# loop-Z/omniisaacgymenvs_loop

Hardware: AMD Instinct MI355X
Metric: env-steps/sec USV_CaptureXY at 1/2/4/8 MI355X; wall-clock to reward=30 (higher is better)
Workload: dtype fp32; 1 GPU; USV_Virtual_CaptureXY num_envs=131072/GPU PPO-MLP fp32 (BASELINE configs[4] per GPU: 2^20 envs over 8 GPUs); num_envs_per_gpu=131072, horizon_length=16, minibatch_size=8192, mini_epochs=8, parallelism=dp1, exchange=none (one rank), seed=0, full=False

## Files before the change

omniisaacgymenvs_loop_amd/csrc/ppo.hip:

```cpp
#include <cstdlib>
#include <cstring>
#include <type_traits>

#include "usv_device.h"

USV_PROBE_DEFINE(ppo)
USV_PROBE_DEFINE(pol)
USV_PROBE_DEFINE(red)

namespace {

constexpr int NIN = PPO_NIN, NH = PPO_NH, NA = PPO_NA;
constexpr int RB = 32;
constexpr int TB = 256;
constexpr int XS = 35;
constexpr int HS = 129;
constexpr int NPART = PPO_NPARAM + 8;
constexpr int NPART_PAD = (NPART + 3) & ~3;
constexpr int P_LOSS = PPO_NPARAM;
constexpr float kLog2Pi = 1.8378770664093453f;

typedef float f32x16 __attribute__((ext_vector_type(16)));
typedef unsigned int u32x4_t __attribute__((ext_vector_type(4)));

// ... 831 lines not shown
    double *o = part + ((size_t)mb * OM_CH + ch) * 2 * NIN;
    o[tid] = t;
    o[NIN + tid] = t2;
  }
}

constexpr int RS_TB = 256, RS_U = 8;
__global__ __launch_bounds__(RS_TB) void k_obs_rms_seq(ppo_cfg_t c, const double *__restrict__ part, int nmb,
                                                       double *obs_rms, double *seq) {
  const double rows = (double)c.minibatch;
  for (int q = threadIdx.x; q < nmb * NIN; q += RS_TB) {
    const int mb = q / NIN, k = q % NIN;
    double sa = 0, sb = 0;
#pragma unroll
    for (int ch = 0; ch < OM_CH; ++ch) {
      const double *o = part + ((size_t)mb * OM_CH + ch) * 2 * NIN;
      sa += o[k];
      sb += o[NIN + k];
    }
    const double bmean = sa / rows;
    seq[(size_t)mb * 2 * NIN + k] = bmean;
    seq[(size_t)mb * 2 * NIN + NIN + k] = (sb - rows * bmean * bmean) / (rows - 1.0);
  }
  __syncthreads();
  const int k = threadIdx.x;
  if (k < NIN) {
    double mean = obs_rms[k], var = obs_rms[NIN + k], count = obs_rms[2 * NIN];
    for (int mb0 = 0; mb0 < nmb; mb0 += RS_U) {
      double bm[RS_U], bv[RS_U];
#pragma unroll
      for (int u = 0; u < RS_U; ++u) {
        const int mb = min(mb0 + u, nmb - 1);
        bm[u] = seq[(size_t)mb * 2 * NIN + k];
        bv[u] = seq[(size_t)mb * 2 * NIN + NIN + k];
      }
#pragma unroll
      for (int u = 0; u < RS_U; ++u) {
        if (mb0 + u >= nmb) break;
        const double tot = count + rows;
        const double delta = bm[u] - mean;
        const double M2 = var * count + bv[u] * rows + delta * delta * count * rows / tot;
        mean = mean + delta * rows / tot;
        var = M2 / tot;
        count = tot;
        seq[(size_t)(mb0 + u) * 2 * NIN + k] = mean;
        seq[(size_t)(mb0 + u) * 2 * NIN + NIN + k] = var;
      }
    }
    obs_rms[k] = mean;
    obs_rms[NIN + k] = var;
    if (k == 0) obs_rms[2 * NIN] = count;
  }
}

constexpr int GTB = 512;
#ifndef USV_BWD_SYNC
#define USV_BWD_SYNC 0
#endif
#ifndef USV_BWD_PRIO
#define USV_BWD_PRIO 0
#endif

#ifndef USV_RD_P
#define USV_RD_P 128
#endif
#ifndef USV_RD_NT
#define USV_RD_NT 1
#endif
typedef float f32x4v __attribute__((ext_vector_type(4)));
constexpr int RD_TB = 512, RD_P = USV_RD_P;
constexpr int RD_L = RD_P / 4;
constexpr int RD_G = (RD_TB / RD_L);
constexpr int RD_KB = 16;
constexpr int RED_BLOCKS = (PPO_NPARAM + 5 + RD_P - 1) / RD_P;
static_assert(RD_P % 4 == 0 && 64 % RD_L == 0 && RD_P <= RD_TB, "reduce geometry");
static_assert(RED_BLOCKS <= 256, "chunk squares: one per thread of waves 0-3");

struct AdamBanks {
  const float *P0, *m0, *v0;
  float *P1, *m1, *v1;
};
struct AdamK {
  float step_size, bc2s;
};
__device__ __forceinline__ AdamK adam_consts(const ppo_cfg_t &c, float lr, float step) {
  const double bc1 = 1.0 - pow((double)c.adam_b1, (double)step);
  const double bc2 = 1.0 - pow((double)c.adam_b2, (double)step);
  return {(float)((double)lr / bc1), (float)sqrt(bc2)};
}
__device__ __forceinline__ void adam_one(const ppo_cfg_t &c, const AdamK &k, float g, float p_old, float m_old,
                                         float v_old, float &pn, float &mn, float &vn) {
  if (c.weight_decay != 0.f) g = g + c.weight_decay * p_old;
  mn = m_old + (1.0f - c.adam_b1) * (g - m_old);
  vn = v_old * c.adam_b2 + (1.0f - c.adam_b2) * g * g;
  const float denom = sqrtf(vn) / k.bc2s + c.adam_eps;
  pn = p_old - k.step_size * (mn / denom);
}
__device__ __forceinline__ float clip_coef(const ppo_cfg_t &c, float total_norm) {
  float coef = 1.0f;
  if (c.truncate_grads) {
    coef = c.grad_norm / (total_norm + 1e-6f);
    coef = fminf(coef, 1.0f);
  }
  return coef;
}
__device__ __forceinline__ AdamK adam_consts_tagged(const ppo_cfg_t &c, float lr, float step, float t_ss,
                                                    float t_bc, float t_step, float t_lr) {
  if (t_step == step && t_lr == lr) return {t_ss, t_bc};
  return adam_consts(c, lr, step);
}
struct OptNext {
  float nl, kl_keep, step;
  AdamK nk;
};
template <class OptIn>
__device__ __forceinline__ OptNext opt_next(const ppo_cfg_t &c, const OptIn &opt_in, float kl) {
  const float lr = opt_in[0];
  float nl = lr, kl_keep = opt_in[2];
  if (c.lr_adaptive) {
    if (kl > 2.0f * c.kl_threshold) nl = fmaxf(lr / 1.5f, c.lr_min);
    if (kl < 0.5f * c.kl_threshold) nl = fminf(lr * 1.5f, c.lr_max);
    kl_keep = kl;
  }
  const float step = opt_in[1] + 1.0f;
  return {nl, kl_keep, step, adam_consts(c, nl, step + 1.0f)};
}
__device__ __forceinline__ void opt_store(const ppo_cfg_t &c, const OptNext &x, float *opt_out, float total_norm,
                                          float kl, float *kl_out) {
  if (c.lr_adaptive && kl_out) *kl_out = kl;
  opt_out[0] = x.nl;
  opt_out[1] = x.step;
  opt_out[2] = x.kl_keep;
  opt_out[3] = total_norm;
  opt_out[4] = x.nk.step_size;
  opt_out[5] = x.nk.bc2s;
  opt_out[6] = x.step + 1.0f;
  opt_out[7] = x.nl;
}

struct ChainIn {
  const float *P_prev, *m_prev, *v_prev;
  float *P_cur, *m_cur, *v_cur;
  const float *grad;
  const float *opt_prev;
  float *opt_cur;
  float *kl_out;
  uint32_t *dp_clock;
  int fold_skip;
  float gscale;
};

constexpr int XG = XS;
constexpr int GX = ((RB * XG + GTB - 1) / GTB) * GTB;
struct GradSmem {
  float w2[NH * HS];
  float w1[NH * XG];
  float x[GX];
  float h1[RB * HS];
  float h2[RB * HS];
  float xch[4][16][64];
  float out[RB * 4];
  float g[RB * 4];
  float hg[4][4][NH];
  float b1[NH];
  float tail[TAIL + 1];
  float nrm[4];
  int fold[2];
};

constexpr int S_W2 = 0, S_W1 = NH * NH, S_SIG = S_W1 + NH * 32, S_B1 = S_SIG + 2, S_TAIL = S_B1 + NH,
              S_W1C = S_TAIL + TAIL, S_END = S_W1C + NH;
static_assert(S_END == PPO_NPARAM && S_W1 % 4 == 0 && NIN == 33, "partial slot layout");
__device__ __forceinline__ int tail_slot(int param) { return S_TAIL + param - PPO_OFF_B2; }
__device__ __forceinline__ int acc_slot(int base, int tile, int a, int lane) { return base + ((tile * 4 + a) * 64 + lane) * 4; }
__device__ __forceinline__ int param_of_slot(int s) {
  if (s < S_W1) {
    const int tile = s >> 10, a = (s >> 8) & 3, lane = (s >> 2) & 63, q = 4 * a + (s & 3);
    const int n = 32 * (tile >> 2) + crow(q, lane >> 5), k = 32 * (tile & 3) + (lane & 31);
    return PPO_OFF_W2 + n * NH + k;
  }
  if (s < S_SIG) {
    const int t = s - S_W1, tile = t >> 10, a = (t >> 8) & 3, lane = (t >> 2) & 63, q = 4 * a + (t & 3);
    const int n = 32 * tile + crow(q, lane >> 5), k = lane & 31;
    return PPO_OFF_W1 + n * NIN + k;
  }
  if (s < S_B1) return PPO_OFF_SIGMA + (s - S_SIG);
  if (s < S_TAIL) return PPO_OFF_B1 + (s - S_B1);
  if (s < S_W1C) return PPO_OFF_B2 + (s - S_TAIL);
  if (s < S_END) return PPO_OFF_W1 + (s - S_W1C) * NIN + (NIN - 1);
  return -1;
}

#ifndef USV_ROW_NT
#define USV_ROW_NT 0
#endif
__device__ __forceinline__ float row_ld(const float *p) {
  if constexpr (USV_ROW_NT != 0) return __builtin_nontemporal_load(p);
  else return *p;
}
struct RowIn {
  float act0, act1, nlp, val, ret, adv, mu0, mu1, sg0, sg1;
};

#ifndef USV_PART_AUX
#define USV_PART_AUX 2
#endif
template <int kAux, bool kCM>
struct PartOutT {
  __amdgpu_buffer_rsrc_t r;
  uint32_t cs;
  __device__ __forceinline__ uint32_t off(int idx) const {
    if constexpr (kCM) return (uint32_t)(idx / RD_P) * cs + (uint32_t)(idx % RD_P) * 4u;
    else return (uint32_t)idx * 4u;
  }
  __device__ __forceinline__ void operator()(int idx, float v) const {
    __builtin_amdgcn_raw_buffer_store_b32(__builtin_bit_cast(uint32_t, v), r, off(idx), 0, kAux);
  }
  __device__ __forceinline__ void x4(int idx, float a, float b, float c, float d) const {
    const u32x4_t v = {__builtin_bit_cast(uint32_t, a), __builtin_bit_cast(uint32_t, b), __builtin_bit_cast(uint32_t, c),
                       __builtin_bit_cast(uint32_t, d)};
    __builtin_amdgcn_raw_buffer_store_b128(v, r, off(idx), 0, kAux);
  }
};
#ifndef USV_PART_CM
#define USV_PART_CM 1
#endif
constexpr int AUX_SC1 = 16;

constexpr int FOLD_G = 8;
static_assert(RD_G >= FOLD_G, "k_reduce_partials(fold = 1) reads one group row per row group");
constexpr int FOLD_MAX_M = 32;
constexpr int FOLD_CTL_STRIDE = 64;
constexpr uint64_t FOLD_WAIT_TICKS = 10000;
__host__ __device__ constexpr size_t part_body_floats(int nblk) {
  return (size_t)nblk * RED_BLOCKS * RD_P > (size_t)(nblk + FOLD_G) * NPART_PAD ? (size_t)nblk * RED_BLOCKS * RD_P
                                                                                 : (size_t)(nblk + FOLD_G) * NPART_PAD;
}
__device__ __forceinline__ uint32_t *fold_ctl(float *partials, int nblk) {
  return reinterpret_cast<uint32_t *>(partials + part_body_floats(nblk));
}
__device__ __forceinline__ const uint32_t *fold_ctl(const float *partials, int nblk) {
  return reinterpret_cast<const uint32_t *>(partials + part_body_floats(nblk));
}
__device__ __forceinline__ f32x4v ld4_sc1(__amdgpu_buffer_rsrc_t r, uint32_t byte_off) {
  return __builtin_bit_cast(f32x4v, __builtin_amdgcn_raw_buffer_load_b128(r, byte_off, 0, AUX_SC1));
}

__device__ __forceinline__ void redo_step(const ppo_cfg_t &c, const ChainIn &ch, const float (&op)[8], float coef,
                                          float scale, GradSmem &s, float &ls0, float &ls1) {
  const AdamK ak = adam_consts_tagged(c, op[0], op[1] + 1.0f, op[4], op[5], op[6], op[7]);
  for (int q = threadIdx.x; q < PPO_NPARAM; q += GTB) {
    float pn, mn, vn;
    adam_one(c, ak, ch.grad[q] * scale * coef, ch.P_prev[q], ch.m_prev[q], ch.v_prev[q], pn, mn, vn);
    if ((q / GTB) % gridDim.x == blockIdx.x) {
      ch.P_cur[q] = pn; ch.m_cur[q] = mn; ch.v_cur[q] = vn;
    }
    if (q >= PPO_OFF_B2) {
      s.tail[q - PPO_OFF_B2] = pn;
    } else if (q >= PPO_OFF_W2) {
      const int e = q - PPO_OFF_W2;
      s.w2[(e / NH) * HS + e % NH] = pn;
    } else if (q >= PPO_OFF_B1) {
      s.b1[q - PPO_OFF_B1] = pn;
    } else if (q >= PPO_OFF_W1) {
      const int e = q - PPO_OFF_W1;
      s.w1[(e / NIN) * XG + e % NIN] = pn;
    }
  }
  float pn, mn, vn;
  adam_one(c, ak, ch.grad[PPO_OFF_SIGMA] * scale * coef, ch.P_prev[PPO_OFF_SIGMA], ch.m_prev[PPO_OFF_SIGMA],
           ch.v_prev[PPO_OFF_SIGMA], pn, mn, vn);
  ls0 = pn;
  adam_one(c, ak, ch.grad[PPO_OFF_SIGMA + 1] * scale * coef, ch.P_prev[PPO_OFF_SIGMA + 1],
           ch.m_prev[PPO_OFF_SIGMA + 1], ch.v_prev[PPO_OFF_SIGMA + 1], pn, mn, vn);
  ls1 = pn;
}

constexpr int APN_TB = 256;
__device__ __forceinline__ float apply_norm_part(const float *__restrict__ grad_in, float grad_scale, int tid) {
  constexpr int N4 = PPO_NPARAM / 4, U = (N4 + APN_TB - 1) / APN_TB;
  const float4 *g4 = reinterpret_cast<const float4 *>(grad_in);
  float4 gv[U];
#pragma unroll
  for (int u = 0; u < U; ++u) gv[u] = g4[min(tid + u * APN_TB, N4 - 1)];
  float ss = 0.f;
#pragma unroll
  for (int u = 0; u < U; ++u) {
    if (tid + u * APN_TB >= N4) continue;
    const float x = gv[u].x * grad_scale, y = gv[u].y * grad_scale;
    const float z = gv[u].z * grad_scale, w = gv[u].w * grad_scale;
    ss = fmaf(x, x, ss); ss = fmaf(y, y, ss); ss = fmaf(z, z, ss); ss = fmaf(w, w, ss);
  }
  for (int r = 4 * N4 + tid; r < PPO_NPARAM; r += APN_TB) {
    const float g = grad_in[r] * grad_scale;
    ss = fmaf(g, g, ss);
  }
  return ss;
}

template <bool kBf, bool kChain, bool kFold, bool kColl = false>
__device__ __forceinline__ void mb_grad8w(const ppo_cfg_t &c, const ChainIn &ch, const float *__restrict__ P,
                                          const double *__restrict__ obs_rms, int row0,
                                          const float *__restrict__ e_obs, const float *__restrict__ e_act,
                                          const float *__restrict__ e_nlp, const float *__restrict__ e_val,
                                          const float *__restrict__ e_ret, const float *__restrict__ e_adv,
                                          float *e_mu, float *e_sigma, float *partials, GradSmem &s) {
  const int tid = threadIdx.x, lane = tid & 63, w = tid >> 6;
  const int i = lane & 31, h = lane >> 5;
  const int kh = w >> 2, cb = w & 3, n0 = 32 * cb;
#ifdef USV_DIAG_HOT_ROWS
  const int rb0 = blockIdx.x * RB;
#else
  const int rb0 = row0 + blockIdx.x * RB;
#endif
  const float invB = 1.0f / (float)c.minibatch;
  USV_PHASE(ppo, 0);
  if (ch.dp_clock && blockIdx.x == 0 && tid == 0) *ch.dp_clock += 1u;
  constexpr int NW1G = (NH * XG + GTB - 1) / GTB, NTLG = (TAIL + GTB - 1) / GTB, NW2F = NH * NH / GTB;
  static_assert(NH * NH % GTB == 0, "staging trip counts");
  float w2f[NW2F];
  float w1r[NW1G], tlr[NTLG];
  float ov = 0.f;
  if constexpr (kChain) ov = lane < 8 ? ch.opt_prev[lane] : ch.grad[PPO_NPARAM];
  {
#pragma unroll
    for (int u = 0; u < NW1G; ++u) {
      const int q = min(tid + u * GTB, NH * XG - 1), j = q / XG, k = q % XG;
      w1r[u] = P[PPO_OFF_W1 + j * NIN + min(k, NIN - 1)];
    }
#pragma unroll
    for (int u = 0; u < NTLG; ++u) tlr[u] = P[PPO_OFF_B2 + min(tid + u * GTB, TAIL - 1)];
  }
  const float b1r = P[PPO_OFF_B1 + (tid & (NH - 1))];
  const float lsv = P[PPO_OFF_SIGMA + (lane & 1)];
  float lsig0 = 0.f, lsig1 = 0.f;
  float csq = 0.f;
  if constexpr (kChain) csq = ch.grad[PPO_NPARAM + 8 + min(tid, RED_BLOCKS - 1)];
  RowIn ri;
  {
    const size_t row = (size_t)rb0 + (lane & (RB - 1));
    ri.act0 = row_ld(&e_act[row * 2]); ri.act1 = row_ld(&e_act[row * 2 + 1]);
    ri.nlp = row_ld(&e_nlp[row]); ri.adv = row_ld(&e_adv[row]);
    ri.val = row_ld(&e_val[row]); ri.ret = row_ld(&e_ret[row]);
    ri.mu0 = row_ld(&e_mu[row * 2]); ri.mu1 = row_ld(&e_mu[row * 2 + 1]);
    ri.sg0 = row_ld(&e_sigma[row * 2]); ri.sg1 = row_ld(&e_sigma[row * 2 + 1]);
  }
  constexpr int NU = (RB * XG + GTB - 1) / GTB;
  float xo[NU];
  double mu[NU], var[NU];
#pragma unroll
  for (int u = 0; u < NU; ++u) {
    const int q = min(tid + u * GTB, RB * XG - 1), r = q / XG, kc = min(q % XG, NIN - 1);
    xo[u] = row_ld(&e_obs[(size_t)(rb0 + r) * NIN + kc]);
    mu[u] = obs_rms[kc];
    var[u] = obs_rms[NIN + kc];
  }
#pragma unroll
  for (int u = 0; u < NW2F; ++u) w2f[u] = P[PPO_OFF_W2 + tid + u * GTB];
  __builtin_amdgcn_sched_barrier(0);
#pragma unroll
  for (int u = 0; u < NW1G; ++u)
    if ((tid + u * GTB) % XG >= NIN) w1r[u] = 0.f;
  if (kChain && tid >= RED_BLOCKS) csq = 0.f;
  {
    const bool norm = c.normalize_input != 0;
#pragma unroll
    for (int u = 0; u < NU; ++u) {
      const int q = tid + u * GTB;
      const int k = q % XG;
      const float xn = rms_norm(xo[u], mu[u], var[u], c.rms_eps);
      const float xv = (k < NIN && q < RB * XG) ? (norm ? xn : xo[u]) : 0.f;
      s.x[q] = xv;
    }
  }
#pragma unroll
  for (int u = 0; u < NW1G; ++u)
    if (tid + u * GTB < NH * XG) s.w1[tid + u * GTB] = w1r[u];
#pragma unroll
  for (int u = 0; u < NTLG; ++u)
    if (tid + u * GTB < TAIL) s.tail[tid + u * GTB] = tlr[u];
  if (tid < NH) s.b1[tid] = b1r;
  if (kChain && !kColl && w < 4) {
    const float t = wave_sum(csq);
    if (lane == 0) s.nrm[w] = t;
  }
  __syncthreads();
  if constexpr (kColl) {
    if (w < 4) {
      const float t = wave_sum(apply_norm_part(ch.grad, ch.gscale, tid));
      if (lane == 0) s.nrm[w] = t;
    }
    __syncthreads();
  }
  bool slow = false;
  if constexpr (kChain) {
    const auto lane_of = [&](int q) {
      return __builtin_bit_cast(float, __builtin_amdgcn_readlane(__builtin_bit_cast(int, ov), q));
    };
    const float total_norm = sqrtf(((s.nrm[0] + s.nrm[1]) + s.nrm[2]) + s.nrm[3]);
    const float coef = clip_coef(c, total_norm);
    const float gscale = kColl ? ch.gscale : 1.0f;
    if (blockIdx.x == 0 && tid == 256) {
      float op[8];
#pragma unroll
      for (int q = 0; q < 8; ++q) op[q] = lane_of(q);
      const float kl_prev = kColl ? lane_of(8) * gscale : lane_of(8);
      opt_store(c, opt_next(c, op, kl_prev), ch.opt_cur, total_norm, kl_prev, ch.kl_out);
    }
    if (kColl || coef < 1.0f) {
      slow = true;
      float op[8];
#pragma unroll
      for (int q = 0; q < 8; ++q) op[q] = lane_of(q);
      redo_step(c, ch, op, coef, gscale, s, lsig0, lsig1);
      __syncthreads();
    }
  }
  USV_PHASE(ppo, 1);
  if (kh == 0) {
    f32x16 acc = {};
#pragma unroll
    for (int st = 0; st < 17; ++st) {
      const int k = 2 * st + h;
      acc = mfma32(s.x[i * XG + k], s.w1[(n0 + i) * XG + k], acc);
    }
    const float bj = s.b1[n0 + i];
#pragma unroll
    for (int r = 0; r < 16; ++r) s.h1[crow(r, h) * HS + n0 + i] = fast_tanh(acc[r] + bj);
  }
  USV_PHASE(ppo, 9);
  if (!slow) {
#pragma unroll
    for (int u = 0; u < NW2F; ++u) {
      const int e = tid + u * GTB;
      s.w2[(e >> 7) * HS + (e & (NH - 1))] = w2f[u];
    }
  }
  __syncthreads();
  USV_PHASE(ppo, 10);
  const int ra = (i + 16 * kh) & (RB - 1);
  {
    f32x16 acc = {};
    if constexpr (kBf) {
#pragma unroll
      for (int st = 0; st < NH / 32; ++st) {
        const int k0 = 64 * kh + 16 * st + 8 * h;
        acc = mfma_bf16(ld8(&s.h1[ra * HS + k0]), ld8(&s.w2[(n0 + i) * HS + k0]), acc);
      }
    } else {
#pragma unroll 16
      for (int st = 0; st < NH / 4; ++st) {
        const int k = 64 * kh + 2 * st + h;
        acc = mfma32(s.h1[ra * HS + k], s.w2[(n0 + i) * HS + k], acc);
      }
    }
    USV_PHASE(ppo, 11);
#pragma unroll
    for (int q = 0; q < 8; ++q) s.xch[cb][8 * kh + q][lane] = acc[8 + q];
    __syncthreads();
    const float bj = s.tail[T_B2 + n0 + i];
#pragma unroll
    for (int q = 0; q < 8; ++q)
      s.h2[(crow(q, h) + 16 * kh) * HS + n0 + i] = fast_tanh((acc[q] + s.xch[cb][8 - 8 * kh + q][lane]) + bj);
  }
  __syncthreads();
  USV_PHASE(ppo, 12);
  constexpr bool kCM = USV_PART_CM != 0 && !kFold;
  const PartOutT<kFold ? AUX_SC1 : USV_PART_AUX, kCM> part_st{
      kCM ? __builtin_amdgcn_make_buffer_rsrc(partials + (size_t)blockIdx.x * RD_P, 0,
                                              (int)(((size_t)RED_BLOCKS * gridDim.x - blockIdx.x) * RD_P * 4), 0x00020000)
          : __builtin_amdgcn_make_buffer_rsrc(partials + (size_t)blockIdx.x * NPART_PAD, 0, NPART * 4, 0x00020000),
      (uint32_t)gridDim.x * RD_P * 4u};
  {
    const int r = tid / 16, part = tid % 16;
    float a0 = 0.f, a1 = 0.f, av = 0.f;
#pragma unroll
    for (int kk = 0; kk < 8; ++kk) {
      const int k = part + 16 * kk;
      const float hv = s.h2[r * HS + k];
      a0 = fmaf(s.tail[T_WMU + k], hv, a0);
      a1 = fmaf(s.tail[T_WMU + NH + k], hv, a1);
      av = fmaf(s.tail[T_WV + k], hv, av);
    }
#pragma unroll
    for (int m = 1; m < 16; m <<= 1) {
      a0 += __shfl_xor(a0, m, 64);
      a1 += __shfl_xor(a1, m, 64);
      av += __shfl_xor(av, m, 64);
    }
    if (part == 0) {
      s.out[r * 4 + 0] = a0 + s.tail[T_BMU];
      s.out[r * 4 + 1] = a1 + s.tail[T_BMU + 1];
      s.out[r * 4 + 2] = av + s.tail[T_BV];
    }
  }
  __syncthreads();
  USV_PHASE(ppo, 2);
  if (tid < 192) {
    const int r = lane;
    const bool rowok = r < RB;
    const int rr = rowok ? r : 0;
    const size_t row = (size_t)rb0 + rr;
    const float mu0 = s.out[rr * 4], mu1 = s.out[rr * 4 + 1], v = s.out[rr * 4 + 2];
    if (!slow) {
      lsig0 = __builtin_bit_cast(float, __builtin_amdgcn_readlane(__builtin_bit_cast(int, lsv), 0));
      lsig1 = __builtin_bit_cast(float, __builtin_amdgcn_readlane(__builtin_bit_cast(int, lsv), 1));
    }
    const float ls0 = mu0 * 0.f + lsig0, ls1 = mu1 * 0.f + lsig1;
    const float sg0 = expf(ls0), sg1 = expf(ls1);
    const float bh0 = fmaxf(mu0 - 1.1f, 0.f), bl0 = fminf(mu0 + 1.1f, 0.f);
    const float bh1 = fmaxf(mu1 - 1.1f, 0.f), bl1 = fminf(mu1 + 1.1f, 0.f);
    if (w == 0) {
      float la = 0.f, gs0 = 0.f, gs1 = 0.f;
      if (rowok) {
        const float z0 = (ri.act0 - mu0) / sg0, z1 = (ri.act1 - mu1) / sg1;
        const float nlp = 0.5f * (z0 * z0 + z1 * z1) + kLog2Pi + (ls0 + ls1);
        const float A = ri.adv;
        const float ratio = expf(ri.nlp - nlp);
        const float lo = 1.0f - c.e_clip, hi = 1.0f + c.e_clip;
        const float rc = clampt(ratio, lo, hi);
        const float s1 = -(A * ratio), s2 = -(A * rc);
        const float a_loss = fmaxf(s1, s2);
        const float inr = (ratio >= lo && ratio <= hi) ? 1.f : 0.f;
        const float g1 = -A, g2 = -A * inr;
        const float g_r = (s1 > s2) ? g1 : ((s1 < s2) ? g2 : 0.5f * (g1 + g2));
        const float dnlp = invB * g_r * (-ratio);
        const float bc = c.bounds_loss_coef * invB;
        const float dmu0 = dnlp * (-z0 / sg0) + bc * 2.f * (bh0 + bl0);
        const float dmu1 = dnlp * (-z1 / sg1) + bc * 2.f * (bh1 + bl1);
        const float dent = -c.entropy_coef * invB;
        gs0 = dnlp * (1.f - z0 * z0) + dent;
        gs1 = dnlp * (1.f - z1 * z1) + dent;
        la = a_loss;
        s.g[r * 4 + 0] = dmu0;
        s.g[r * 4 + 1] = dmu1;
        s.g[r * 4 + 3] = dnlp;
      }
      la = wave_sum(la); gs0 = wave_sum(gs0); gs1 = wave_sum(gs1);
      if (lane == 0) {
        part_st(P_LOSS + 0, la);
        part_st(S_SIG, gs0); part_st(S_SIG + 1, gs1);
      }
    } else if (w == 2) {
      float le = 0.f, lb = 0.f, lkl = 0.f;
      if (rowok) {
        const float b_loss = (bl0 * bl0 + bh0 * bh0) + (bl1 * bl1 + bh1 * bh1);
        const float ent = (0.5f + 0.5f * logf(USV_2PI_F) + ls0) + (0.5f + 0.5f * logf(USV_2PI_F) + ls1);
        const float om0 = ri.mu0, om1 = ri.mu1, os0 = ri.sg0, os1 = ri.sg1;
        const float kl0 = logf(os0 / sg0 + 1e-5f) + (sg0 * sg0 + (om0 - mu0) * (om0 - mu0)) / (2.0f * (os0 * os0 + 1e-5f)) - 0.5f;
        const float kl1 = logf(os1 / sg1 + 1e-5f) + (sg1 * sg1 + (om1 - mu1) * (om1 - mu1)) / (2.0f * (os1 * os1 + 1e-5f)) - 0.5f;
        e_mu[row * 2] = mu0; e_mu[row * 2 + 1] = mu1;
        e_sigma[row * 2] = sg0; e_sigma[row * 2 + 1] = sg1;
        le = ent; lb = b_loss; lkl = kl0 + kl1;
      }
      le = wave_sum(le); lb = wave_sum(lb); lkl = wave_sum(lkl);
      if (lane == 0) {
        part_st(P_LOSS + 2, le); part_st(P_LOSS + 3, lb); part_st(P_LOSS + 4, lkl);
      }
    } else {
      float lc = 0.f;
      if (rowok) {
        const float vo = ri.val, R = ri.ret;
        float dv, c_loss;
        if (c.clip_value) {
          const float dvr = v - vo;
          const float dvc = clampt(dvr, -c.e_clip, c.e_clip);
          const float vc = vo + dvc;
          const float l1 = (v - R) * (v - R), l2 = (vc - R) * (vc - R);
          c_loss = fmaxf(l1, l2);
          const float d1 = 2.f * (v - R);
          const float d2 = 2.f * (vc - R) * ((dvr >= -c.e_clip && dvr <= c.e_clip) ? 1.f : 0.f);
          dv = (l1 > l2) ? d1 : ((l1 < l2) ? d2 : 0.5f * (d1 + d2));
        } else {
          c_loss = (R - v) * (R - v);
          dv = 2.f * (v - R);
        }
        dv *= 0.5f * c.critic_coef * invB;
        lc = c_loss;
        s.g[r * 4 + 2] = dv;
      }
      lc = wave_sum(lc);
      if (lane == 0) part_st(P_LOSS + 1, lc);
    }
  }
  __syncthreads();
  USV_PHASE(ppo, 3);
  {
    const int j = tid & (NH - 1), qq = tid >> 7;
    const float wm0 = s.tail[T_WMU + j], wm1 = s.tail[T_WMU + NH + j], wv = s.tail[T_WV + j];
    float gw0 = 0.f, gw1 = 0.f, gwv = 0.f, db = 0.f;
#pragma unroll
    for (int q = 0; q < RB / 4; ++q) {
      const int rr = qq * (RB / 4) + q;
      const float hv = s.h2[rr * HS + j];
      const float d0 = s.g[rr * 4], d1 = s.g[rr * 4 + 1], dvv = s.g[rr * 4 + 2];
      gw0 = fmaf(d0, hv, gw0); gw1 = fmaf(d1, hv, gw1); gwv = fmaf(dvv, hv, gwv);
      const float dz = (d0 * wm0 + d1 * wm1 + dvv * wv) * (1.f - hv * hv);
      s.h2[rr * HS + j] = dz;
      db += dz;
    }
    s.hg[qq][0][j] = gw0; s.hg[qq][1][j] = gw1; s.hg[qq][2][j] = gwv; s.hg[qq][3][j] = db;
  }
  __syncthreads();
  USV_PHASE(ppo, 4);
  f32x16 dh = {};
  if (w < 4) {
    if constexpr (USV_BWD_PRIO > 0) __builtin_amdgcn_s_setprio(USV_BWD_PRIO);
    if constexpr (kBf) {
#pragma unroll
      for (int st = 0; st < NH / 16; ++st) {
        const int j0 = 16 * st + 8 * h;
        dh = mfma_bf16(ld8(&s.h2[i * HS + j0]), ld8s(&s.w2[j0 * HS + n0 + i], HS), dh);
      }
    } else {
#pragma unroll 16
      for (int st = 0; st < NH / 2; ++st) {
        const int j = 2 * st + h;
        dh = mfma32(s.h2[i * HS + j], s.w2[j * HS + n0 + i], dh);
      }
    }
    USV_PHASE(ppo, 6);
  } else {
    const int tt = tid - 256;
    if (tt < NH) {
      const int j = tt;
      part_st(tail_slot(PPO_OFF_WMU + j), ((s.hg[0][0][j] + s.hg[1][0][j]) + s.hg[2][0][j]) + s.hg[3][0][j]);
      part_st(tail_slot(PPO_OFF_WMU + NH + j), ((s.hg[0][1][j] + s.hg[1][1][j]) + s.hg[2][1][j]) + s.hg[3][1][j]);
      part_st(tail_slot(PPO_OFF_WV + j), ((s.hg[0][2][j] + s.hg[1][2][j]) + s.hg[2][2][j]) + s.hg[3][2][j]);
      part_st(tail_slot(PPO_OFF_B2 + j), ((s.hg[0][3][j] + s.hg[1][3][j]) + s.hg[2][3][j]) + s.hg[3][3][j]);
    } else if (tt < NH + 3) {
      const int q = tt - NH;
      float sacc = 0.f;
      for (int r = 0; r < RB; ++r) sacc += s.g[r * 4 + q];
      part_st(tail_slot(q < 2 ? PPO_OFF_BMU + q : PPO_OFF_BV), sacc);
    }
  }
  if constexpr (USV_BWD_SYNC != 0) __syncthreads();
  if (w < 4) {
    float dz1[16];
#pragma unroll
    for (int q = 0; q < 16; ++q) {
      const float hv = s.h1[crow(q, h) * HS + n0 + i];
      dz1[q] = dh[q] * (1.f - hv * hv);
    }
    USV_PHASE(ppo, 7);
    f32x16 acc = {};
#pragma unroll
    for (int q = 0; q < 16; ++q) acc = mfma32(dz1[q], s.x[crow(q, h) * XG + i], acc);
    float sb = 0.f, sc = 0.f;
#pragma unroll
    for (int q = 0; q < 16; ++q) {
      sb += dz1[q];
      sc = fmaf(dz1[q], s.x[crow(q, h) * XG + NIN - 1], sc);
    }
    sb += __shfl_xor(sb, 32, 64);
    sc += __shfl_xor(sc, 32, 64);
#pragma unroll
    for (int a = 0; a < 4; ++a)
      part_st.x4(acc_slot(S_W1, cb, a, lane), acc[4 * a], acc[4 * a + 1], acc[4 * a + 2], acc[4 * a + 3]);
    if (h == 0) {
      part_st(S_B1 + n0 + i, sb);
      part_st(S_W1C + n0 + i, sc);
    }
  } else {
    const int t = w - 4;
    const int nt0 = 32 * t;
    {
    f32x16 prev = {};
#pragma unroll
    for (int kb = 0; kb < 4; ++kb) {
      f32x16 d = {};
      if constexpr (kBf) {
#pragma unroll
        for (int st = 0; st < RB / 16; ++st) {
          const int r0 = 16 * st + 8 * h;
          d = mfma_bf16(ld8s(&s.h2[r0 * HS + nt0 + i], HS), ld8s(&s.h1[r0 * HS + 32 * kb + i], HS), d);
          if (kb > 0) {
#pragma unroll
            for (int a = 2 * st; a < 2 * st + 2; ++a)
              part_st.x4(acc_slot(S_W2, 4 * t + kb - 1, a, lane), prev[4 * a], prev[4 * a + 1], prev[4 * a + 2],
                         prev[4 * a + 3]);
            __builtin_amdgcn_sched_barrier(0);
          }
        }
      } else {
#pragma unroll
        for (int st = 0; st < RB / 2; ++st) {
          const int r = st + 16 * h;
          d = mfma32(s.h2[r * HS + nt0 + i], s.h1[r * HS + 32 * kb + i], d);
          if (kb > 0 && (st & 3) == 1) {
            const int a = st >> 2;
            part_st.x4(acc_slot(S_W2, 4 * t + kb - 1, a, lane), prev[4 * a], prev[4 * a + 1], prev[4 * a + 2],
                       prev[4 * a + 3]);
            __builtin_amdgcn_sched_barrier(0);
          }
        }
      }
      prev = d;
    }
    USV_PHASE_T(ppo, 13, 256);
#pragma unroll
    for (int a = 0; a < 4; ++a)
      part_st.x4(acc_slot(S_W2, 4 * t + 3, a, lane), prev[4 * a], prev[4 * a + 1], prev[4 * a + 2], prev[4 * a + 3]);
    USV_PHASE_T(ppo, 5, 256);
    }
  }
  USV_PHASE(ppo, 8);
  if constexpr (kFold) {
    __asm__ volatile("s_waitcnt vmcnt(0)" ::: "memory");
    __syncthreads();
    const int nblk = (int)gridDim.x, M = nblk / FOLD_G, g = blockIdx.x % FOLD_G, m = blockIdx.x / FOLD_G;
    uint32_t *ctl = fold_ctl(partials, nblk) + g * FOLD_CTL_STRIDE;
    if (tid == 0) {
      __builtin_amdgcn_fence(__ATOMIC_RELEASE, "agent");
      const uint32_t old = __hip_atomic_fetch_add(ctl, 1u, __ATOMIC_RELAXED, __HIP_MEMORY_SCOPE_AGENT);
      const uint32_t gen = old / (uint32_t)M + 1u, target = gen * (uint32_t)M;
      const uint64_t t0 = wall_clock64();
      int ok = 0;
      while (true) {
        const uint32_t v = __hip_atomic_load(ctl, __ATOMIC_RELAXED, __HIP_MEMORY_SCOPE_AGENT);
        if ((int32_t)(v - target) >= 0) { ok = 1; __builtin_amdgcn_fence(__ATOMIC_ACQUIRE, "agent"); break; }
        if (wall_clock64() - t0 > FOLD_WAIT_TICKS) break;
        __builtin_amdgcn_s_sleep(1);
      }
      s.fold[0] = ok && !ch.fold_skip;
      s.fold[1] = (int)gen;
    }
    __syncthreads();
    USV_PHASE(ppo, 14);
    if (s.fold[0]) {
      constexpr int NQ = NPART_PAD / 4;
      const int q4 = (NQ + M - 1) / M, qa = m * q4, qb = min(qa + q4, NQ);
      const int h0 = (M + 1) / 2;
      float4 *lds = reinterpret_cast<float4 *>(s.w2);
      const __amdgpu_buffer_rsrc_t rows = __builtin_amdgcn_make_buffer_rsrc(
          partials + (size_t)g * NPART_PAD, 0, (int)((size_t)(nblk - g) * NPART_PAD * 4), 0x00020000);
      float *grow = partials + (size_t)(nblk + g) * NPART_PAD;
      for (int c0 = qa; c0 < qb; c0 += GTB / 2) {
        const int half = tid / (GTB / 2), q = c0 + tid % (GTB / 2);
        const int mb = half ? h0 : 0, me = half ? M : h0;
        const int qc = min(q, NQ - 1);
        f32x4v x[FOLD_MAX_M / 2];
#pragma unroll
        for (int k = 0; k < FOLD_MAX_M / 2; ++k)
          x[k] = ld4_sc1(rows, (uint32_t)((FOLD_G * min(mb + k, M - 1) * NPART_PAD + 4 * qc) * 4));
        f32x4v acc = {0.f, 0.f, 0.f, 0.f};
#pragma unroll
        for (int k = 0; k < FOLD_MAX_M / 2; ++k)
          if (mb + k < me) acc += x[k];
        if (half) lds[tid % (GTB / 2)] = make_float4(acc[0], acc[1], acc[2], acc[3]);
        __syncthreads();
        if (!half && q < qb) {
          const float4 o = lds[tid];
          const f32x4v t = {acc[0] + o.x, acc[1] + o.y, acc[2] + o.z, acc[3] + o.w};
          __builtin_nontemporal_store(t, reinterpret_cast<f32x4v *>(grow + 4 * q));
        }
        __syncthreads();
      }
      __asm__ volatile("s_waitcnt vmcnt(0)" ::: "memory");
      __syncthreads();
      if (tid == 0) ctl[32 + m] = (uint32_t)s.fold[1];
    }
    USV_PHASE(ppo, 15);
  }
}

template <bool kBf, bool kChain, bool kFold, bool kColl = false>
__global__ __launch_bounds__(GTB, 2) void k_mb_grad(ppo_cfg_t c, ChainIn ch, const float *__restrict__ P,
                                                    const double *__restrict__ obs_rms, int row0,
                                                    const float *__restrict__ e_obs, const float *__restrict__ e_act,
                                                    const float *__restrict__ e_nlp, const float *__restrict__ e_val,
                                                    const float *__restrict__ e_ret, const float *__restrict__ e_adv,
                                                    float *e_mu, float *e_sigma, float *partials) {
  __shared__ GradSmem s;
  mb_grad8w<kBf, kChain, kFold, kColl>(c, ch, P, obs_rms, row0, e_obs, e_act, e_nlp, e_val, e_ret, e_adv, e_mu,
                                       e_sigma, partials, s);
}

constexpr int DP_SLOTS = RED_BLOCKS * RD_P;
constexpr int DP_FLAG_STRIDE = 32;
constexpr long long DP_X_BYTES = 2LL * PPO_DP_MAX * DP_SLOTS * 4;
constexpr long long DP_FLAG_OFF = (DP_X_BYTES + 4095) / 4096 * 4096;
constexpr long long DP_BYTES = DP_FLAG_OFF + (long long)RED_BLOCKS * PPO_DP_MAX * DP_FLAG_STRIDE * 4;
__device__ __forceinline__ void st_sys(float *p, float v) {
  __hip_atomic_store(reinterpret_cast<uint32_t *>(p), __builtin_bit_cast(uint32_t, v), __ATOMIC_RELAXED,
                     __HIP_MEMORY_SCOPE_SYSTEM);
}
__device__ __forceinline__ float ld_sys(const float *p) {
  return __builtin_bit_cast(float, __hip_atomic_load(reinterpret_cast<const uint32_t *>(p), __ATOMIC_RELAXED,
                                                     __HIP_MEMORY_SCOPE_SYSTEM));
}
__device__ __forceinline__ float *dp_x(void *buf, int par, int sender) {
  return reinterpret_cast<float *>(buf) + ((size_t)par * PPO_DP_MAX + sender) * DP_SLOTS;
}
__device__ __forceinline__ uint32_t *dp_flag(void *buf, int chunk, int sender) {
  return reinterpret_cast<uint32_t *>(reinterpret_cast<char *>(buf) + DP_FLAG_OFF) +
         ((size_t)chunk * PPO_DP_MAX + sender) * DP_FLAG_STRIDE;
}

#ifndef USV_DP_ORDER
#define USV_DP_ORDER 2
#endif
__device__ float dp_exchange(const ppo_dp_t &dp, uint32_t key, int chunk, int slot, float pv, int timeout_ms) {
  const int tid = threadIdx.x, lane = tid & 63, w = tid >> 6;
  const int par = (int)(key & 1u);
  if (tid < RD_P)
    for (int r = 0; r < dp.world; ++r) st_sys(dp_x(dp.peer[r], par, dp.rank) + slot, pv);
  __asm__ volatile("s_waitcnt vmcnt(0)" ::: "memory");
  __syncthreads();
  if (w == 0) {
    if (lane < dp.world) {
      if constexpr ((USV_DP_ORDER & 1) != 0) {
        __builtin_amdgcn_fence(__ATOMIC_RELEASE, "");
        __asm__ volatile("s_waitcnt vmcnt(0)" ::: "memory");
        __hip_atomic_store(dp_flag(dp.peer[lane], chunk, dp.rank), key, __ATOMIC_RELAXED, __HIP_MEMORY_SCOPE_SYSTEM);
      } else {
        __hip_atomic_store(dp_flag(dp.peer[lane], chunk, dp.rank), key, __ATOMIC_RELAXED, __HIP_MEMORY_SCOPE_SYSTEM);
      }
    }
    const uint64_t t0 = wall_clock64(), lim = (uint64_t)timeout_ms * 100000ull;
    bool got = lane >= dp.world;
    while (true) {
      if (!got) {
        const uint32_t f = __hip_atomic_load(dp_flag(dp.peer[dp.rank], chunk, lane), __ATOMIC_RELAXED,
                                             __HIP_MEMORY_SCOPE_SYSTEM);
        got = (int32_t)(f - key) >= 0;
      }
      if (__all(got)) break;
      const int32_t e = __hip_atomic_load(dp.err, __ATOMIC_RELAXED, __HIP_MEMORY_SCOPE_AGENT);
      if (e != 0) break;
      if (wall_clock64() - t0 > lim) {
        if (lane == 0) atomicOr(dp.err, 1);
        break;
      }
      __builtin_amdgcn_s_sleep(2);
    }
    if constexpr ((USV_DP_ORDER & 2) != 0) {
      __builtin_amdgcn_fence(__ATOMIC_ACQUIRE, "");
      __asm__ volatile("s_waitcnt vmcnt(0)" ::: "memory");
    }
  }
  __syncthreads();
  float t = 0.f;
  if (tid < RD_P) {
    const float *xs = dp_x(dp.peer[dp.rank], par, 0);
    for (int r = 0; r < dp.world; ++r) t += ld_sys(xs + (size_t)r * DP_SLOTS + slot);
  }
  return t;
}

__device__ __forceinline__ float dp_probe_value(int sender, int round, int slot) {
  return (float)(sender * 1000003 + round * 65537 + slot);
}
__global__ __launch_bounds__(RD_TB) void k_dp_selftest(ppo_dp_t dp, uint32_t key0, int rounds, int timeout_ms) {
  const int tid = threadIdx.x;
  const int slot = blockIdx.x * RD_P + tid;
  for (int rd = 0; rd < rounds; ++rd) {
// ... 541 lines not shown
```

Before: 35.72 million env-steps/s.

## Fuse PPO head forward/loss per row-group and defer tail-gradient reduction to idle waves

Restructures the fused PPO gradient kernel's second-layer and head stages. Each K-half of the layer-2 MFMA now writes its partial sum to its own shared buffer (h2 and a new bank-skewed z2u), which replaces the xch exchange and one barrier. The 16 threads that own a row then apply bias and tanh, compute the head outputs with shuffles, and evaluate the actor and critic losses and gradients in registers, which removes the out/g/hg buffers and several __syncthreads. The head-weight and bias gradient sums and the entropy/KL losses move to waves 4-7 after the backward MFMA work, so they run alongside it. In exchange there is more register pressure and redundant per-thread loss math (16 threads per row), and the row inputs are loaded in a different pattern.

Result: faster. 36.13 million env-steps/s (median of 6 runs) (+1.1%).

```diff
diff --git a/omniisaacgymenvs_loop_amd/csrc/ppo.hip b/omniisaacgymenvs_loop_amd/csrc/ppo.hip
--- a/omniisaacgymenvs_loop_amd/csrc/ppo.hip
+++ b/omniisaacgymenvs_loop_amd/csrc/ppo.hip
@@ -1007,16 +1007,16 @@
 
 constexpr int XG = XS;
 constexpr int GX = ((RB * XG + GTB - 1) / GTB) * GTB;
+enum { RV_LA, RV_LC, RV_GS0, RV_GS1, RV_DMU0, RV_DMU1, RV_DV, RV_MU0, RV_MU1, RV_N };
+__device__ __forceinline__ int z2u_at(int row, int k) { return row * NH + ((k + 16 * (row & 1)) & (NH - 1)); }
 struct GradSmem {
   float w2[NH * HS];
   float w1[NH * XG];
   float x[GX];
   float h1[RB * HS];
   float h2[RB * HS];
-  float xch[4][16][64];
-  float out[RB * 4];
-  float g[RB * 4];
-  float hg[4][4][NH];
+  float z2u[RB * NH];
+  float rowv[RV_N][RB];
   float b1[NH];
   float tail[TAIL + 1];
   float nrm[4];
@@ -1193,12 +1193,12 @@
   if constexpr (kChain) csq = ch.grad[PPO_NPARAM + 8 + min(tid, RED_BLOCKS - 1)];
   RowIn ri;
   {
-    const size_t row = (size_t)rb0 + (lane & (RB - 1));
+    const size_t row = (size_t)rb0 + (tid >> 4), rowl = (size_t)rb0 + (lane & (RB - 1));
     ri.act0 = row_ld(&e_act[row * 2]); ri.act1 = row_ld(&e_act[row * 2 + 1]);
     ri.nlp = row_ld(&e_nlp[row]); ri.adv = row_ld(&e_adv[row]);
     ri.val = row_ld(&e_val[row]); ri.ret = row_ld(&e_ret[row]);
-    ri.mu0 = row_ld(&e_mu[row * 2]); ri.mu1 = row_ld(&e_mu[row * 2 + 1]);
-    ri.sg0 = row_ld(&e_sigma[row * 2]); ri.sg1 = row_ld(&e_sigma[row * 2 + 1]);
+    ri.mu0 = row_ld(&e_mu[rowl * 2]); ri.mu1 = row_ld(&e_mu[rowl * 2 + 1]);
+    ri.sg0 = row_ld(&e_sigma[rowl * 2]); ri.sg1 = row_ld(&e_sigma[rowl * 2 + 1]);
   }
   constexpr int NU = (RB * XG + GTB - 1) / GTB;
   float xo[NU];
@@ -1293,30 +1293,29 @@
   }
   __syncthreads();
   USV_PHASE(ppo, 10);
-  const int ra = (i + 16 * kh) & (RB - 1);
   {
     f32x16 acc = {};
     if constexpr (kBf) {
 #pragma unroll
       for (int st = 0; st < NH / 32; ++st) {
         const int k0 = 64 * kh + 16 * st + 8 * h;
-        acc = mfma_bf16(ld8(&s.h1[ra * HS + k0]), ld8(&s.w2[(n0 + i) * HS + k0]), acc);
+        acc = mfma_bf16(ld8(&s.h1[i * HS + k0]), ld8(&s.w2[(n0 + i) * HS + k0]), acc);
       }
     } else {
 #pragma unroll 16
       for (int st = 0; st < NH / 4; ++st) {
         const int k = 64 * kh + 2 * st + h;
-        acc = mfma32(s.h1[ra * HS + k], s.w2[(n0 + i) * HS + k], acc);
+        acc = mfma32(s.h1[i * HS + k], s.w2[(n0 + i) * HS + k], acc);
       }
     }
     USV_PHASE(ppo, 11);
-#pragma unroll
-    for (int q = 0; q < 8; ++q) s.xch[cb][8 * kh + q][lane] = acc[8 + q];
-    __syncthreads();
-    const float bj = s.tail[T_B2 + n0 + i];
-#pragma unroll
-    for (int q = 0; q < 8; ++q)
-      s.h2[(crow(q, h) + 16 * kh) * HS + n0 + i] = fast_tanh((acc[q] + s.xch[cb][8 - 8 * kh + q][lane]) + bj);
+    if (kh == 0) {
+#pragma unroll
+      for (int q = 0; q < 16; ++q) s.h2[crow(q, h) * HS + n0 + i] = acc[q];
+    } else {
+#pragma unroll
+      for (int q = 0; q < 16; ++q) s.z2u[z2u_at(crow(q, h), n0 + i)] = acc[q];
+    }
   }
   __syncthreads();
   USV_PHASE(ppo, 12);
@@ -1326,16 +1325,19 @@
                                               (int)(((size_t)RED_BLOCKS * gridDim.x - blockIdx.x) * RD_P * 4), 0x00020000)
           : __builtin_amdgcn_make_buffer_rsrc(partials + (size_t)blockIdx.x * NPART_PAD, 0, NPART * 4, 0x00020000),
       (uint32_t)gridDim.x * RD_P * 4u};
+  const int r = tid >> 4, part = tid & 15;
+  float hv[8], wm0[8], wm1[8], wv[8];
+  float mu0, mu1, v;
   {
-    const int r = tid / 16, part = tid % 16;
     float a0 = 0.f, a1 = 0.f, av = 0.f;
 #pragma unroll
     for (int kk = 0; kk < 8; ++kk) {
       const int k = part + 16 * kk;
-      const float hv = s.h2[r * HS + k];
-      a0 = fmaf(s.tail[T_WMU + k], hv, a0);
-      a1 = fmaf(s.tail[T_WMU + NH + k], hv, a1);
-      av = fmaf(s.tail[T_WV + k], hv, av);
+      hv[kk] = fast_tanh((s.h2[r * HS + k] + s.z2u[z2u_at(r, k)]) + s.tail[T_B2 + k]);
+      wm0[kk] = s.tail[T_WMU + k]; wm1[kk] = s.tail[T_WMU + NH + k]; wv[kk] = s.tail[T_WV + k];
+      a0 = fmaf(wm0[kk], hv[kk], a0);
+      a1 = fmaf(wm1[kk], hv[kk], a1);
+      av = fmaf(wv[kk], hv[kk], av);
     }
 #pragma unroll
     for (int m = 1; m < 16; m <<= 1) {
@@ -1343,20 +1345,12 @@
       a1 += __shfl_xor(a1, m, 64);
       av += __shfl_xor(av, m, 64);
     }
-    if (part == 0) {
-      s.out[r * 4 + 0] = a0 + s.tail[T_BMU];
-      s.out[r * 4 + 1] = a1 + s.tail[T_BMU + 1];
-      s.out[r * 4 + 2] = av + s.tail[T_BV];
-    }
-  }
-  __syncthreads();
+    mu0 = a0 + s.tail[T_BMU];
+    mu1 = a1 + s.tail[T_BMU + 1];
+    v = av + s.tail[T_BV];
+  }
   USV_PHASE(ppo, 2);
-  if (tid < 192) {
-    const int r = lane;
-    const bool rowok = r < RB;
-    const int rr = rowok ? r : 0;
-    const size_t row = (size_t)rb0 + rr;
-    const float mu0 = s.out[rr * 4], mu1 = s.out[rr * 4 + 1], v = s.out[rr * 4 + 2];
+  {
     if (!slow) {
       lsig0 = __builtin_bit_cast(float, __builtin_amdgcn_readlane(__builtin_bit_cast(int, lsv), 0));
       lsig1 = __builtin_bit_cast(float, __builtin_amdgcn_readlane(__builtin_bit_cast(int, lsv), 1));
@@ -1365,99 +1359,60 @@
     const float sg0 = expf(ls0), sg1 = expf(ls1);
     const float bh0 = fmaxf(mu0 - 1.1f, 0.f), bl0 = fminf(mu0 + 1.1f, 0.f);
     const float bh1 = fmaxf(mu1 - 1.1f, 0.f), bl1 = fminf(mu1 + 1.1f, 0.f);
-    if (w == 0) {
-      float la = 0.f, gs0 = 0.f, gs1 = 0.f;
-      if (rowok) {
-        const float z0 = (ri.act0 - mu0) / sg0, z1 = (ri.act1 - mu1) / sg1;
-        const float nlp = 0.5f * (z0 * z0 + z1 * z1) + kLog2Pi + (ls0 + ls1);
-        const float A = ri.adv;
-        const float ratio = expf(ri.nlp - nlp);
-        const float lo = 1.0f - c.e_clip, hi = 1.0f + c.e_clip;
-        const float rc = clampt(ratio, lo, hi);
-        const float s1 = -(A * ratio), s2 = -(A * rc);
-        const float a_loss = fmaxf(s1, s2);
-        const float inr = (ratio >= lo && ratio <= hi) ? 1.f : 0.f;
-        const float g1 = -A, g2 = -A * inr;
-        const float g_r = (s1 > s2) ? g1 : ((s1 < s2) ? g2 : 0.5f * (g1 + g2));
-        const float dnlp = invB * g_r * (-ratio);
-        const float bc = c.bounds_loss_coef * invB;
-        const float dmu0 = dnlp * (-z0 / sg0) + bc * 2.f * (bh0 + bl0);
-        const float dmu1 = dnlp * (-z1 / sg1) + bc * 2.f * (bh1 + bl1);
-        const float dent = -c.entropy_coef * invB;
-        gs0 = dnlp * (1.f - z0 * z0) + dent;
-        gs1 = dnlp * (1.f - z1 * z1) + dent;
-        la = a_loss;
-        s.g[r * 4 + 0] = dmu0;
-        s.g[r * 4 + 1] = dmu1;
-        s.g[r * 4 + 3] = dnlp;
-      }
-      la = wave_sum(la); gs0 = wave_sum(gs0); gs1 = wave_sum(gs1);
-      if (lane == 0) {
-        part_st(P_LOSS + 0, la);
-        part_st(S_SIG, gs0); part_st(S_SIG + 1, gs1);
-      }
-    } else if (w == 2) {
-      float le = 0.f, lb = 0.f, lkl = 0.f;
-      if (rowok) {
-        const float b_loss = (bl0 * bl0 + bh0 * bh0) + (bl1 * bl1 + bh1 * bh1);
-        const float ent = (0.5f + 0.5f * logf(USV_2PI_F) + ls0) + (0.5f + 0.5f * logf(USV_2PI_F) + ls1);
-        const float om0 = ri.mu0, om1 = ri.mu1, os0 = ri.sg0, os1 = ri.sg1;
-        const float kl0 = logf(os0 / sg0 + 1e-5f) + (sg0 * sg0 + (om0 - mu0) * (om0 - mu0)) / (2.0f * (os0 * os0 + 1e-5f)) - 0.5f;
-        const float kl1 = logf(os1 / sg1 + 1e-5f) + (sg1 * sg1 + (om1 - mu1) * (om1 - mu1)) / (2.0f * (os1 * os1 + 1e-5f)) - 0.5f;
-        e_mu[row * 2] = mu0; e_mu[row * 2 + 1] = mu1;
-        e_sigma[row * 2] = sg0; e_sigma[row * 2 + 1] = sg1;
-        le = ent; lb = b_loss; lkl = kl0 + kl1;
-      }
-      le = wave_sum(le); lb = wave_sum(lb); lkl = wave_sum(lkl);
-      if (lane == 0) {
-        part_st(P_LOSS + 2, le); part_st(P_LOSS + 3, lb); part_st(P_LOSS + 4, lkl);
-      }
-    } else {
-      float lc = 0.f;
-      if (rowok) {
-        const float vo = ri.val, R = ri.ret;
-        float dv, c_loss;
-        if (c.clip_value) {
-          const float dvr = v - vo;
-          const float dvc = clampt(dvr, -c.e_clip, c.e_clip);
-          const float vc = vo + dvc;
-          const float l1 = (v - R) * (v - R), l2 = (vc - R) * (vc - R);
-          c_loss = fmaxf(l1, l2);
-          const float d1 = 2.f * (v - R);
-          const float d2 = 2.f * (vc - R) * ((dvr >= -c.e_clip && dvr <= c.e_clip) ? 1.f : 0.f);
-          dv = (l1 > l2) ? d1 : ((l1 < l2) ? d2 : 0.5f * (d1 + d2));
-        } else {
-          c_loss = (R - v) * (R - v);
-          dv = 2.f * (v - R);
-        }
-        dv *= 0.5f * c.critic_coef * invB;
-        lc = c_loss;
-        s.g[r * 4 + 2] = dv;
-      }
-      lc = wave_sum(lc);
-      if (lane == 0) part_st(P_LOSS + 1, lc);
-    }
-  }
-  __syncthreads();
-  USV_PHASE(ppo, 3);
-  {
-    const int j = tid & (NH - 1), qq = tid >> 7;
-    const float wm0 = s.tail[T_WMU + j], wm1 = s.tail[T_WMU + NH + j], wv = s.tail[T_WV + j];
-    float gw0 = 0.f, gw1 = 0.f, gwv = 0.f, db = 0.f;
-#pragma unroll
-    for (int q = 0; q < RB / 4; ++q) {
-      const int rr = qq * (RB / 4) + q;
-      const float hv = s.h2[rr * HS + j];
-      const float d0 = s.g[rr * 4], d1 = s.g[rr * 4 + 1], dvv = s.g[rr * 4 + 2];
-      gw0 = fmaf(d0, hv, gw0); gw1 = fmaf(d1, hv, gw1); gwv = fmaf(dvv, hv, gwv);
-      const float dz = (d0 * wm0 + d1 * wm1 + dvv * wv) * (1.f - hv * hv);
-      s.h2[rr * HS + j] = dz;
-      db += dz;
-    }
-    s.hg[qq][0][j] = gw0; s.hg[qq][1][j] = gw1; s.hg[qq][2][j] = gwv; s.hg[qq][3][j] = db;
-  }
-  __syncthreads();
-  USV_PHASE(ppo, 4);
+    float dmu0, dmu1, dv, la, lc, gs0, gs1;
+    {
+      const float z0 = (ri.act0 - mu0) / sg0, z1 = (ri.act1 - mu1) / sg1;
+      const float nlp = 0.5f * (z0 * z0 + z1 * z1) + kLog2Pi + (ls0 + ls1);
+      const float A = ri.adv;
+      const float ratio = expf(ri.nlp - nlp);
+      const float lo = 1.0f - c.e_clip, hi = 1.0f + c.e_clip;
+      const float rc = clampt(ratio, lo, hi);
+      const float s1 = -(A * ratio), s2 = -(A * rc);
+      la = fmaxf(s1, s2);
+      const float inr = (ratio >= lo && ratio <= hi) ? 1.f : 0.f;
+      const float g1 = -A, g2 = -A * inr;
+      const float g_r = (s1 > s2) ? g1 : ((s1 < s2) ? g2 : 0.5f * (g1 + g2));
+      const float dnlp = invB * g_r * (-ratio);
+      const float bc = c.bounds_loss_coef * invB;
+      dmu0 = dnlp * (-z0 / sg0) + bc * 2.f * (bh0 + bl0);
+      dmu1 = dnlp * (-z1 / sg1) + bc * 2.f * (bh1 + bl1);
+      const float dent = -c.entropy_coef * invB;
+      gs0 = dnlp * (1.f - z0 * z0) + dent;
+      gs1 = dnlp * (1.f - z1 * z1) + dent;
+    }
+    {
+      const float vo = ri.val, R = ri.ret;
+      if (c.clip_value) {
+        const float dvr = v - vo;
+        const float dvc = clampt(dvr, -c.e_clip, c.e_clip);
+        const float vc = vo + dvc;
+        const float l1 = (v - R) * (v - R), l2 = (vc - R) * (vc - R);
+        lc = fmaxf(l1, l2);
+        const float d1 = 2.f * (v - R);
+        const float d2 = 2.f * (vc - R) * ((dvr >= -c.e_clip && dvr <= c.e_clip) ? 1.f : 0.f);
+        dv = (l1 > l2) ? d1 : ((l1 < l2) ? d2 : 0.5f * (d1 + d2));
+      } else {
+        lc = (R - v) * (R - v);
+        dv = 2.f * (v - R);
+      }
+      dv *= 0.5f * c.critic_coef * invB;
+    }
+    USV_PHASE(ppo, 3);
+#pragma unroll
+    for (int kk = 0; kk < 8; ++kk) {
+      const int k = part + 16 * kk;
+      s.h2[r * HS + k] = (dmu0 * wm0[kk] + dmu1 * wm1[kk] + dv * wv[kk]) * (1.f - hv[kk] * hv[kk]);
+    }
+    USV_PHASE(ppo, 4);
+#pragma unroll
+    for (int kk = 0; kk < 8; ++kk) s.z2u[z2u_at(r, part + 16 * kk)] = hv[kk];
+    if (part == 0) {
+      s.rowv[RV_LA][r] = la; s.rowv[RV_LC][r] = lc; s.rowv[RV_GS0][r] = gs0; s.rowv[RV_GS1][r] = gs1;
+      s.rowv[RV_DMU0][r] = dmu0; s.rowv[RV_DMU1][r] = dmu1; s.rowv[RV_DV][r] = dv;
+      s.rowv[RV_MU0][r] = mu0; s.rowv[RV_MU1][r] = mu1;
+    }
+  }
+  __syncthreads();
   f32x16 dh = {};
   if (w < 4) {
     if constexpr (USV_BWD_PRIO > 0) __builtin_amdgcn_s_setprio(USV_BWD_PRIO);
@@ -1475,20 +1430,6 @@
       }
     }
     USV_PHASE(ppo, 6);
-  } else {
-    const int tt = tid - 256;
-    if (tt < NH) {
-      const int j = tt;
-      part_st(tail_slot(PPO_OFF_WMU + j), ((s.hg[0][0][j] + s.hg[1][0][j]) + s.hg[2][0][j]) + s.hg[3][0][j]);
-      part_st(tail_slot(PPO_OFF_WMU + NH + j), ((s.hg[0][1][j] + s.hg[1][1][j]) + s.hg[2][1][j]) + s.hg[3][1][j]);
-      part_st(tail_slot(PPO_OFF_WV + j), ((s.hg[0][2][j] + s.hg[1][2][j]) + s.hg[2][2][j]) + s.hg[3][2][j]);
-      part_st(tail_slot(PPO_OFF_B2 + j), ((s.hg[0][3][j] + s.hg[1][3][j]) + s.hg[2][3][j]) + s.hg[3][3][j]);
-    } else if (tt < NH + 3) {
-      const int q = tt - NH;
-      float sacc = 0.f;
-      for (int r = 0; r < RB; ++r) sacc += s.g[r * 4 + q];
-      part_st(tail_slot(q < 2 ? PPO_OFF_BMU + q : PPO_OFF_BV), sacc);
-    }
   }
   if constexpr (USV_BWD_SYNC != 0) __syncthreads();
   if (w < 4) {
@@ -1558,6 +1499,66 @@
     for (int a = 0; a < 4; ++a)
       part_st.x4(acc_slot(S_W2, 4 * t + 3, a, lane), prev[4 * a], prev[4 * a + 1], prev[4 * a + 2], prev[4 * a + 3]);
     USV_PHASE_T(ppo, 5, 256);
+    }
+    const int tt = tid - 256;
+    if (tt < NH) {
+      const int j = tt;
+      float gw0[4], gw1[4], gwv[4], db[4];
+#pragma unroll
+      for (int qq = 0; qq < 4; ++qq) {
+        gw0[qq] = gw1[qq] = gwv[qq] = db[qq] = 0.f;
+#pragma unroll
+        for (int q = 0; q < RB / 4; ++q) {
+          const int rr = qq * (RB / 4) + q;
+          const float hj = s.z2u[z2u_at(rr, j)];
+          gw0[qq] = fmaf(s.rowv[RV_DMU0][rr], hj, gw0[qq]);
+          gw1[qq] = fmaf(s.rowv[RV_DMU1][rr], hj, gw1[qq]);
+          gwv[qq] = fmaf(s.rowv[RV_DV][rr], hj, gwv[qq]);
+          db[qq] += s.h2[rr * HS + j];
+        }
+      }
+      part_st(tail_slot(PPO_OFF_WMU + j), ((gw0[0] + gw0[1]) + gw0[2]) + gw0[3]);
+      part_st(tail_slot(PPO_OFF_WMU + NH + j), ((gw1[0] + gw1[1]) + gw1[2]) + gw1[3]);
+      part_st(tail_slot(PPO_OFF_WV + j), ((gwv[0] + gwv[1]) + gwv[2]) + gwv[3]);
+      part_st(tail_slot(PPO_OFF_B2 + j), ((db[0] + db[1]) + db[2]) + db[3]);
+    } else {
+      const bool rowok = lane < RB;
+      const int rr = lane & (RB - 1);
+      if (w == 6) {
+        const float la = wave_sum(rowok ? s.rowv[RV_LA][rr] : 0.f), gs0 = wave_sum(rowok ? s.rowv[RV_GS0][rr] : 0.f);
+        const float gs1 = wave_sum(rowok ? s.rowv[RV_GS1][rr] : 0.f), lc = wave_sum(rowok ? s.rowv[RV_LC][rr] : 0.f);
+        if (lane == 0) {
+          part_st(P_LOSS + 0, la); part_st(P_LOSS + 1, lc);
+          part_st(S_SIG, gs0); part_st(S_SIG + 1, gs1);
+        } else if (lane < 4) {
+          const int q = lane - 1;
+          float sacc = 0.f;
+          for (int r2 = 0; r2 < RB; ++r2) sacc += s.rowv[RV_DMU0 + q][r2];
+          part_st(tail_slot(q < 2 ? PPO_OFF_BMU + q : PPO_OFF_BV), sacc);
+        }
+      } else {
+        const float m0 = s.rowv[RV_MU0][rr], m1 = s.rowv[RV_MU1][rr];
+        const float ls0 = m0 * 0.f + lsig0, ls1 = m1 * 0.f + lsig1;
+        const float sg0 = expf(ls0), sg1 = expf(ls1);
+        const float bh0 = fmaxf(m0 - 1.1f, 0.f), bl0 = fminf(m0 + 1.1f, 0.f);
+        const float bh1 = fmaxf(m1 - 1.1f, 0.f), bl1 = fminf(m1 + 1.1f, 0.f);
+        float le = 0.f, lb = 0.f, lkl = 0.f;
+        if (rowok) {
+          const size_t row = (size_t)rb0 + rr;
+          const float b_loss = (bl0 * bl0 + bh0 * bh0) + (bl1 * bl1 + bh1 * bh1);
+          const float ent = (0.5f + 0.5f * logf(USV_2PI_F) + ls0) + (0.5f + 0.5f * logf(USV_2PI_F) + ls1);
+          const float om0 = ri.mu0, om1 = ri.mu1, os0 = ri.sg0, os1 = ri.sg1;
+          const float kl0 = logf(os0 / sg0 + 1e-5f) + (sg0 * sg0 + (om0 - m0) * (om0 - m0)) / (2.0f * (os0 * os0 + 1e-5f)) - 0.5f;
+          const float kl1 = logf(os1 / sg1 + 1e-5f) + (sg1 * sg1 + (om1 - m1) * (om1 - m1)) / (2.0f * (os1 * os1 + 1e-5f)) - 0.5f;
+          e_mu[row * 2] = m0; e_mu[row * 2 + 1] = m1;
+          e_sigma[row * 2] = sg0; e_sigma[row * 2 + 1] = sg1;
+          le = ent; lb = b_loss; lkl = kl0 + kl1;
+        }
+        le = wave_sum(le); lb = wave_sum(lb); lkl = wave_sum(lkl);
+        if (lane == 0) {
+          part_st(P_LOSS + 2, le); part_st(P_LOSS + 3, lb); part_st(P_LOSS + 4, lkl);
+        }
+      }
     }
   }
   USV_PHASE(ppo, 8);
```
